# google-deepmind/mujoco_warp

Measured on NVIDIA H100. Metric: env-steps/sec (whole box) on humanoid.xml at nworld=8192 per GPU, higher is better.
Workload: dtype f32

## Files before the change

### mujoco_warp_b200/csrc/k_velocity.cu

```cuda

#include "mjb_fluid.cuh"
#include "mjb_math.cuh"
#include "mjb_muscle.cuh"
#include "mjb_team.cuh"
#include "mjb_types.cuh"

namespace {

struct VelLayout { int qvel, cdof, cinert, cvel, cdofdot, cacc, cfrc, qpas, qbias, qact, qsm, qld, x, af, total; };
__host__ __device__ inline VelLayout vel_layout(const ModelDev& m) {
  VelLayout L;
  int o = 0;
  auto pad = [](int n) { return (n + 3) & ~3; };
  auto take = [&](int n) { int r = o; o += pad(n); return r; };
  L.qpas = take(m.nv); L.qbias = take(m.nv);
  L.qsm = L.qpas; L.x = L.qbias;
  const int a0 = o;
  L.cdof = take(6 * m.nv); L.cinert = take(10 * m.nbody); L.qvel = take(m.nv);
  L.cvel = take(6 * m.nbody); L.cdofdot = take(6 * (m.nv > m.nbody ? m.nv : m.nbody)); L.cacc = take(6 * m.nbody);
  L.cfrc = L.cdofdot;
  if (pad(m.nv) + pad(m.nu) <= L.cvel - L.cinert) { L.qact = L.cinert; L.af = L.cinert + pad(m.nv); }
  else { L.qact = take(m.nv); L.af = take(m.nu); }
  L.qld = a0;
  if (o - a0 < pad(m.qld_total)) o = a0 + pad(m.qld_total);
  L.total = o;
  return L;
}

template <int LPW>
__device__ __forceinline__ void team_chol_upper(float* U, int n, float* x, bool solve, int sub) {
#pragma unroll 1
  for (int j = 0; j < n; j++) {
    const int iend = solve ? n + 1 : n;
#pragma unroll 1
    for (int i = j + sub; i < iend; i += LPW) {
      const bool rhs = i == n;
      const float* col = rhs ? x : U + i;
      const int cs = rhs ? 1 : n;
      float s0 = rhs ? x[j] : U[j * n + i], s1 = 0.f;
      int k = 0;
#pragma unroll 4
      for (; k + 1 < j; k += 2) {
        s0 -= U[k * n + j] * col[k * cs];
        s1 -= U[(k + 1) * n + j] * col[(k + 1) * cs];
      }
      if (k < j) s0 -= U[k * n + j] * col[k * cs];
      if (rhs) x[j] = s0 + s1; else U[j * n + i] = s0 + s1;
    }
    __syncwarp();
    const float piv = sqrtf(fmaxf(U[j * n + j], MJ_MINVAL)), inv = 1.0f / piv;
    __syncwarp();
#pragma unroll 1
    for (int i = j + sub; i < iend; i += LPW) {
      if (i == n) x[j] *= inv;
      else U[j * n + i] = i == j ? piv : U[j * n + i] * inv;
    }
    __syncwarp();
  }
  if (!solve) return;
#pragma unroll 1
  for (int j = n - 1; j >= 0; j--) {
    const float xj = x[j] / U[j * n + j];
    __syncwarp();
#pragma unroll 1
    for (int k = sub; k < j; k += LPW) x[k] -= U[k * n + j] * xj;
    if (sub == 0) x[j] = xj;
    __syncwarp();
  }
}

template <bool PEXT, int LPW, bool BAT>
__global__ void __launch_bounds__(256)
k_velocity(const __grid_constant__ ModelDev mp, const __grid_constant__ DataDev d, int mask) {
  constexpr bool FLUID = false;
  [[maybe_unused]] constexpr FluidDev f{};
#include "k_velocity_body.cuh"
}

template <int LPW, bool BAT>
__global__ void __launch_bounds__(256)
k_velocity_fluid(const __grid_constant__ ModelDev mp, const __grid_constant__ DataDev d, int mask, const __grid_constant__ FluidDev f) {
  constexpr bool PEXT = true, FLUID = true;
#include "k_velocity_body.cuh"
}

}

template <bool PEXT>
static TeamKernel vel_instance(int lpw, bool bat) {
  if (bat) return k_velocity<PEXT, 32, true>;
  return lpw == 8 ? k_velocity<PEXT, 8, false> : lpw == 16 ? k_velocity<PEXT, 16, false> : k_velocity<PEXT, 32, false>;
}
static bool vel_pext(const ModelDev& m) { return m.has_gravcomp || m.ntendon > 0; }
static TeamKernel vel_kernel(const ModelDev& m, int lpw) { return vel_pext(m) ? vel_instance<true>(lpw, m.batched) : vel_instance<false>(lpw, m.batched); }
using FluidKernel = void (*)(ModelDev, DataDev, int, FluidDev);
static FluidKernel vel_kernel_fluid(const ModelDev& m, int lpw) {
  if (m.batched) return k_velocity_fluid<32, true>;
  return lpw == 8 ? k_velocity_fluid<8, false> : lpw == 16 ? k_velocity_fluid<16, false> : k_velocity_fluid<32, false>;
}

size_t smem_velocity(const ModelDev& m, const DataDev& d, const FluidDev& f) {
  const int words = vel_layout(m).total;
  return f.has_fluid ? team_shape(m, d.wn, words, vel_kernel_fluid).block_bytes : team_shape(m, d.wn, words, vel_kernel).block_bytes;
}
cudaError_t launch_velocity(const ModelDev& m, const DataDev& d, int mask, cudaStream_t s, const FluidDev& f) {
  const int words = vel_layout(m).total;
  return f.has_fluid ? team_launch(m, d, words, vel_kernel_fluid, mask, s, f) : team_launch(m, d, words, vel_kernel, mask, s);
}
cudaError_t resident_worlds_velocity(const ModelDev& m, const DataDev& d, int* worlds, int* shape, const FluidDev& f) {
  const int words = vel_layout(m).total;
  shape[3] = f.has_fluid ? 2 : vel_pext(m) ? 1 : 0;
  return f.has_fluid ? team_resident_worlds(m, d, words, vel_kernel_fluid, worlds, shape) : team_resident_worlds(m, d, words, vel_kernel, worlds, shape);
}
```

### mujoco_warp_b200/csrc/k_velocity_body.cuh

```cuda
  extern __shared__ __align__(16) float smem[];
  constexpr int G = 32 / LPW;
  Team<LPW> T;
  T.init(d.w0, d.wn, d.nworld);
  if (T.nvalid <= 0) return;
  MJB_WORLD_MODEL(T.w)
  const int lane = T.lane, sub = T.sub, g = T.g, nval = T.nvalid;
  const bool valid = T.valid;
  const VelLayout L = vel_layout(mp);
  float* S = smem + (size_t)(threadIdx.x >> 5) * ((size_t)L.total * G + 4);
  Stager st;
  st.init(reinterpret_cast<uint64_t*>(S + (size_t)L.total * G), lane);
  const int nv = m.nv, nb = m.nbody, nu = m.nu;
#define FLD(f, n) (S + (size_t)L.f * G + (size_t)g * (n))
  float *qvel = FLD(qvel, nv), *cdof = FLD(cdof, 6 * nv), *cinert = FLD(cinert, 10 * nb), *cvel = FLD(cvel, 6 * nb), *cdofdot = FLD(cdofdot, 6 * nv),
        *cacc = FLD(cacc, 6 * nb), *cfrc = FLD(cfrc, 6 * nb), *q_passive = FLD(qpas, nv), *q_bias = FLD(qbias, nv), *q_act = FLD(qact, nv),
        *q_smooth = FLD(qsm, nv), *qld = FLD(qld, m.qld_total), *x = FLD(x, nv), *aforce = FLD(af, nu);
  const float* Mw = d.M + (size_t)T.w * m.nC;
#undef FLD
  const size_t wg = (size_t)T.wg0;
#define GLOAD(f, field, n) st.load(S + (size_t)L.f * G, d.field + wg * (size_t)(n), nval * (n))
#define GSTORE(field, f, n) st.store(d.field + wg * (size_t)(n), S + (size_t)L.f * G, nval * (n))
  const size_t wb = (size_t)T.w;
  const bool v_all = mask & STG_VELOCITY;

  GLOAD(qvel, qvel, nv); GLOAD(cdof, cdof, 6 * nv);
  if (v_all || (mask & STG_RNE)) GLOAD(cinert, cinert, 10 * nb);
  constexpr int MREG = 32;
  float mreg[MREG];
  const bool fac = mask & (STG_ACCELERATION | STG_FACTOR_ONLY);
#pragma unroll
  for (int k = 0; k < MREG; k++) { const int e = sub + k * LPW; mreg[k] = (fac && e < m.nC) ? Mw[e] : 0.f; }
  bool any_xfrc = false;
  if (mask & STG_ACCELERATION) {
#pragma unroll 4
    for (int i = sub; i < 6 * nb; i += LPW) any_xfrc |= d.xfrc_applied[wb * 6 * nb + i] != 0.f;
  }
  st.load_wait();

  if (mask & (STG_VELOCITY | STG_COMVEL | STG_PASSIVE | STG_RNE)) {
    if (v_all)
#pragma unroll 1
    for (int a = valid ? sub : nu; a < nu; a += LPW) {
      const int nnz = d.moment_rownnz[wb * nu + a], adr = d.moment_rowadr[wb * nu + a];
      float vel = 0.f;
      for (int k = 0; k < nnz; k++) vel += d.actuator_moment[wb * m.nJmom + adr + k] * qvel[d.moment_colind[wb * m.nJmom + adr + k]];
      d.actuator_velocity[wb * nu + a] = vel;
    }
    if (PEXT && v_all && m.ntendon > 0) {
#pragma unroll 1
      for (int t = valid ? sub : m.ntendon; t < m.ntendon; t += LPW) {
        float vel = 0.f;
        for (int k = m.ten_J_rowadr[t]; k < m.ten_J_rowadr[t] + m.ten_J_rownnz[t]; k++) vel += m.ten_J0[k] * qvel[m.ten_J_colind[k]];
        d.ten_velocity[wb * m.ntendon + t] = vel;
      }
    }
    if (v_all || (mask & STG_COMVEL)) {
    if (sub < 6) cvel[sub] = 0.f;
    __syncwarp();
#pragma unroll 1
    for (int l = 1; l < m.nlevel; l++) {
#pragma unroll 1
      for (int i = m.level_adr[l] + sub; i < m.level_adr[l + 1]; i += LPW) {
        const int b = m.level_body[i], pid = m.body_parentid[b], jntadr = m.body_jntadr[b], jntnum = m.body_jntnum[b];
        int dof = m.body_dofadr[b];
        float cv[6];
#pragma unroll
        for (int k = 0; k < 6; k++) cv[k] = cvel[6 * pid + k];
#pragma unroll 1
        for (int j = jntadr; j < jntadr + jntnum; j++) {
          const int t = m.jnt_type[j];
          if (t == JNT_FREE) {
            for (int q = 0; q < 3; q++) { const float v = qvel[dof + q]; for (int k = 0; k < 6; k++) { cv[k] += cdof[6 * (dof + q) + k] * v; cdofdot[6 * (dof + q) + k] = 0.f; } }
            for (int q = 3; q < 6; q++) motion_cross(cv, cdof + 6 * (dof + q), cdofdot + 6 * (dof + q));
            for (int q = 3; q < 6; q++) { const float v = qvel[dof + q]; for (int k = 0; k < 6; k++) cv[k] += cdof[6 * (dof + q) + k] * v; }
            dof += 6;
          } else if (t == JNT_BALL) {
            for (int q = 0; q < 3; q++) motion_cross(cv, cdof + 6 * (dof + q), cdofdot + 6 * (dof + q));
            for (int q = 0; q < 3; q++) { const float v = qvel[dof + q]; for (int k = 0; k < 6; k++) cv[k] += cdof[6 * (dof + q) + k] * v; }
            dof += 3;
          } else {
            motion_cross(cv, cdof + 6 * dof, cdofdot + 6 * dof);
            const float v = qvel[dof];
            for (int k = 0; k < 6; k++) cv[k] += cdof[6 * dof + k] * v;
            dof += 1;
          }
        }
#pragma unroll
        for (int k = 0; k < 6; k++) cvel[6 * b + k] = cv[k];
      }
      __syncwarp();
    }
    st.store_fence();
    GSTORE(cvel, cvel, 6 * nb); GSTORE(cdof_dot, cdofdot, 6 * nv);
    st.store_commit();
    } else if (mask & STG_RNE) {
      GLOAD(cvel, cvel, 6 * nb); GLOAD(cdofdot, cdof_dot, 6 * nv);
      st.load_wait();
    }

    if (v_all || (mask & STG_PASSIVE)) {
      const bool dsbl_spring = m.disableflags & DSBL_SPRING, dsbl_damper = m.disableflags & DSBL_DAMPER;
      const bool gravcomp = PEXT && m.has_gravcomp && !(m.disableflags & DSBL_GRAVITY) && !(dsbl_spring && dsbl_damper);
      [[maybe_unused]] const bool fluid = FLUID && !(dsbl_spring && dsbl_damper);
      if constexpr (FLUID) if (fluid) {
        const float* cv = (v_all || (mask & STG_COMVEL)) ? cvel : d.cvel + wb * 6 * nb;
        const float *xip = d.xipos + wb * nb * 3, *stc = d.subtree_com + wb * nb * 3;
#pragma unroll 1
        for (int b = sub; b < nb; b += LPW)
          fluid_body_wrench(m, f, b, cv + 6 * b, ld3(xip + 3 * b), d.ximat + (wb * nb + b) * 9, ld3(stc + 3 * m.body_rootid[b]), d.geom_xpos + wb * m.ngeom * 3,
                            d.geom_xmat + wb * m.ngeom * 9, cacc + 6 * b);
        __syncwarp();
      }
#pragma unroll 1
      for (int dd = sub; dd < nv; dd += LPW) {
        const int j = m.dof_jntid[dd], t = m.jnt_type[j];
        float spring = 0.f, damper = 0.f, gc = 0.f;
        if (!(dsbl_spring && dsbl_damper)) {
          const float stiffness = m.jnt_stiffness[j];
          if (stiffness != 0.f && !dsbl_spring) {
            const int qa = m.jnt_qposadr[j], k = dd - m.jnt_dofadr[j];
            if (t == JNT_SLIDE || t == JNT_HINGE) spring = -(d.qpos[wb * m.nq + qa] - m.qpos_spring[qa]) * stiffness;
            else if (!PEXT) {}
            else if (t == JNT_FREE && k < 3) spring = -stiffness * (d.qpos[wb * m.nq + qa + k] - m.qpos_spring[qa + k]);
            else {
              const int ra = t == JNT_FREE ? qa + 3 : qa, kk = t == JNT_FREE ? k - 3 : k;
              const q4 rot = qnormalize(ldq(d.qpos + wb * m.nq + ra)), ref = ldq(m.qpos_spring + ra);
              const q4 qd = qmul(mkq(ref.w, -ref.x, -ref.y, -ref.z), rot);
              const float s2 = sqrtf(qd.x * qd.x + qd.y * qd.y + qd.z * qd.z);
              if (s2 != 0.f) {
                float speed = 2.0f * atan2f(s2, qd.w);
                if (speed > 3.14159265358979f) speed -= 2.0f * 3.14159265358979f;
                spring = -stiffness * (kk == 0 ? qd.x : kk == 1 ? qd.y : qd.z) * (speed / s2);
              }
            }
          }
          const float damping = m.dof_damping[dd];
          if (damping != 0.f && !dsbl_damper) damper = -qvel[dd] * damping;
          if (PEXT && m.ntendon > 0) {
#pragma unroll 1
            for (int tn = 0; tn < m.ntendon; tn++) {
              const float ks = m.tendon_stiffness[tn], kd = m.tendon_damping[tn];
              if ((ks == 0.f || dsbl_spring) && (kd == 0.f || dsbl_damper)) continue;
              const float J = tendon_J_at(m, tn, dd);
              if (J == 0.f) continue;
              if (ks != 0.f && !dsbl_spring) {
                const float len = d.ten_length[wb * m.ntendon + tn], lo = m.tendon_lengthspring[2 * tn], hi = m.tendon_lengthspring[2 * tn + 1];
                const float x = len > hi ? len - hi : (len < lo ? len - lo : 0.f);
                spring += J * (-x * ks);
              }
              if (kd != 0.f && !dsbl_damper) {
                float vel = 0.f;
                for (int k = m.ten_J_rowadr[tn]; k < m.ten_J_rowadr[tn] + m.ten_J_rownnz[tn]; k++) vel += m.ten_J0[k] * qvel[m.ten_J_colind[k]];
                damper += J * (-vel * kd);
              }
            }
          }
        }
        if (gravcomp) {
#pragma unroll 1
          for (int b = 1; b < nb; b++) {
            const float g = m.body_gravcomp[b];
            if (g == 0.f || !m.body_isdofancestor[b * nv + dd]) continue;
            const float sc = -m.body_mass[b] * g;
            const v3 off = ld3(d.xipos + (wb * nb + b) * 3) - ld3(d.subtree_com + (wb * nb + m.body_rootid[b]) * 3);
            const v3 jp = ld3(cdof + 6 * dd + 3) + cross(ld3(cdof + 6 * dd), off);
            gc += sc * (jp.x * m.gravity_x + jp.y * m.gravity_y + jp.z * m.gravity_z);
          }
        }
        float passive = spring + damper + (m.jnt_actgravcomp[j] ? 0.f : gc);
        if constexpr (FLUID) {
          const float fl = fluid ? fluid_project(m, dd, cdof + 6 * dd, cacc, d.xipos + wb * nb * 3, d.subtree_com + wb * nb * 3) : 0.f;
          passive += fl;
          if (valid) f.qfrc_fluid[wb * nv + dd] = fl;
        }
        q_passive[dd] = passive;
        if (valid) {
          d.qfrc_spring[wb * nv + dd] = spring;
          d.qfrc_damper[wb * nv + dd] = damper;
          d.qfrc_gravcomp[wb * nv + dd] = gc;
          d.qfrc_passive[wb * nv + dd] = passive;
        }
      }
    }
    if (v_all || (mask & STG_RNE)) {
    for (int k = sub; k < 6; k += LPW) cacc[k] = k < 3 ? 0.f : ((m.disableflags & DSBL_GRAVITY) ? 0.f : -(k == 3 ? m.gravity_x : k == 4 ? m.gravity_y : m.gravity_z));
    __syncwarp();
#pragma unroll 1
    for (int l = 1; l < m.nlevel; l++) {
#pragma unroll 1
      for (int i = m.level_adr[l] + sub; i < m.level_adr[l + 1]; i += LPW) {
        const int b = m.level_body[i], pid = m.body_parentid[b];
        float a[6];
#pragma unroll
        for (int k = 0; k < 6; k++) a[k] = cacc[6 * pid + k];
#pragma unroll 1
        for (int q = 0; q < m.body_dofnum[b]; q++) {
          const int dof = m.body_dofadr[b] + q;
          const float v = qvel[dof];
#pragma unroll
          for (int k = 0; k < 6; k++) a[k] += cdofdot[6 * dof + k] * v;
        }
#pragma unroll
        for (int k = 0; k < 6; k++) cacc[6 * b + k] = a[k];
      }
      __syncwarp();
    }
    st.store_wait_read();
#pragma unroll 2
    for (int b = sub; b < nb; b += LPW) {
      float f[6] = {0.f, 0.f, 0.f, 0.f, 0.f, 0.f};
      if (b > 0) {
        float iv[6], g[6];
        inert_vec(cinert + 10 * b, cacc + 6 * b, f);
        inert_vec(cinert + 10 * b, cvel + 6 * b, iv);
        motion_cross_force(cvel + 6 * b, iv, g);
#pragma unroll
        for (int k = 0; k < 6; k++) f[k] += g[k];
      }
#pragma unroll
      for (int k = 0; k < 6; k++) cfrc[6 * b + k] = f[k];
    }
    __syncwarp();
#pragma unroll 1
    for (int l = m.nlevel - 2; l >= 0; l--) {
#pragma unroll 1
      for (int i = m.level_adr[l] + sub; i < m.level_adr[l + 1]; i += LPW) {
        const int b = m.level_body[i];
        float acc[6];
#pragma unroll
        for (int k = 0; k < 6; k++) acc[k] = cfrc[6 * b + k];
#pragma unroll 1
        for (int c = m.body_childadr[b]; c < m.body_childadr[b + 1]; c++) {
          const float* cc = cfrc + 6 * m.body_childid[c];
#pragma unroll
          for (int k = 0; k < 6; k++) acc[k] += cc[k];
        }
#pragma unroll
        for (int k = 0; k < 6; k++) cfrc[6 * b + k] = acc[k];
      }
      __syncwarp();
    }
#pragma unroll 1
    for (int dd = sub; dd < nv; dd += LPW) {
      const float v = dot6(cdof + 6 * dd, cfrc + 6 * m.dof_bodyid[dd]);
      q_bias[dd] = v;
    }
    st.store_fence();
    GSTORE(cacc, cacc, 6 * nb); GSTORE(cfrc_int, cfrc, 6 * nb); GSTORE(qfrc_bias, qbias, nv);
    st.store_commit();
    }
  } else if (mask & STG_ACCELERATION) {
    GLOAD(qpas, qfrc_passive, nv); GLOAD(qbias, qfrc_bias, nv);
    st.load_wait();
  }
  __syncwarp();

  if (mask & STG_ACTUATION) {
#pragma unroll 1
    for (int dd = sub; dd < nv; dd += LPW) q_act[dd] = 0.f;
    __syncwarp();
    const bool enabled = nu > 0 && !(m.disableflags & DSBL_ACTUATION);
#pragma unroll 1
    for (int a = sub; a < nu; a += LPW) {
      float force = 0.f;
      if (enabled) {
        float ctrl = d.ctrl[wb * nu + a];
        if (m.actuator_ctrllimited[a] && !(m.disableflags & DSBL_CLAMPCTRL)) ctrl = clampf(ctrl, m.actuator_ctrlrange[2 * a], m.actuator_ctrlrange[2 * a + 1]);
        const float length = d.actuator_length[wb * nu + a], velocity = d.actuator_velocity[wb * nu + a];
        const float *gp = m.actuator_gainprm + 10 * a, *bp = m.actuator_biasprm + 10 * a;
        float gain = 0.f, bias = 0.f;
        if (m.actuator_gaintype[a] == GAIN_FIXED) gain = gp[0];
        else if (m.actuator_gaintype[a] == GAIN_AFFINE) gain = gp[0] + gp[1] * length + gp[2] * velocity;
        else if (m.actuator_gaintype[a] == GAIN_MUSCLE)
          gain = muscle_gain(length, velocity, m.actuator_lengthrange[2 * a], m.actuator_lengthrange[2 * a + 1], m.actuator_acc0[a], gp);
        if (m.actuator_biastype[a] == BIAS_AFFINE) bias = bp[0] + bp[1] * length + bp[2] * velocity;
        else if (m.actuator_biastype[a] == BIAS_MUSCLE)
          bias = muscle_bias(length, m.actuator_lengthrange[2 * a], m.actuator_lengthrange[2 * a + 1], m.actuator_acc0[a], bp);
        float ctrl_act = ctrl;
        if (m.na > 0 && m.actuator_actadr[a] >= 0) {
          const int last = m.actuator_actadr[a] + m.actuator_actnum[a] - 1, dyn = m.actuator_dyntype[a];
          const float act = d.act[wb * m.na + last];
          float act_dot = 0.f;
          if (dyn == DYN_INTEGRATOR) act_dot = ctrl;
          else if (dyn == DYN_FILTER || dyn == DYN_FILTEREXACT) act_dot = (ctrl - act) / fmaxf(m.actuator_dynprm[10 * a], MJ_MINVAL);
          else if (dyn == DYN_MUSCLE) act_dot = muscle_dynamics(ctrl, act, m.actuator_dynprm + 10 * a);
          if (valid) d.act_dot[wb * m.na + last] = act_dot;
          ctrl_act = m.actuator_actearly[a] ? next_act(m, a, act, act_dot, 1.0f, m.actuator_actlimited[a] != 0) : act;
        }
        force = gain * ctrl_act + bias;
        if (m.actuator_forcelimited[a]) force = clampf(force, m.actuator_forcerange[2 * a], m.actuator_forcerange[2 * a + 1]);
      } else if (m.na > 0 && m.actuator_actadr[a] >= 0 && valid) {
        d.act_dot[wb * m.na + m.actuator_actadr[a] + m.actuator_actnum[a] - 1] = 0.f;
      }
      if (valid) d.actuator_force[wb * nu + a] = force;
      aforce[a] = force;
    }
    __syncwarp();
    if (PEXT && enabled && m.ntendon > 0) {
#pragma unroll 1
      for (int t = sub; t < m.ntendon; t += LPW) {
        if (!m.tendon_actfrclimited[t]) continue;
        float total = 0.f;
        for (int b = 0; b < nu; b++) if (m.actuator_trntype[b] == TRN_TENDON && m.actuator_trnid[2 * b] == t) total += aforce[b];
        const float lo = m.tendon_actfrcrange[2 * t], hi = m.tendon_actfrcrange[2 * t + 1];
        const float sc = total < lo ? lo / total : (total > hi ? hi / total : 1.0f);
        if (sc == 1.0f) continue;
        for (int b = 0; b < nu; b++)
          if (m.actuator_trntype[b] == TRN_TENDON && m.actuator_trnid[2 * b] == t) { aforce[b] *= sc; if (valid) d.actuator_force[wb * nu + b] = aforce[b]; }
      }
      __syncwarp();
    }
    if (enabled) {
#pragma unroll 1
      for (int dd = sub; dd < nv; dd += LPW) {
        float q = 0.f;
        for (int k = m.dofact_adr[dd]; k < m.dofact_adr[dd + 1]; k++) q += d.actuator_moment[wb * m.nJmom + m.dofact_mom[k]] * aforce[m.dofact_act[k]];
        const int j = m.dof_jntid[dd];
        if (!(m.disableflags & DSBL_GRAVITY) && m.jnt_actgravcomp[j]) q += d.qfrc_gravcomp[wb * nv + dd];
        if (m.jnt_actfrclimited[j]) q = clampf(q, m.jnt_actfrcrange[2 * j], m.jnt_actfrcrange[2 * j + 1]);
        q_act[dd] = q;
      }
    }
    st.store_fence();
    GSTORE(qfrc_actuator, qact, nv);
    st.store_commit();
  } else if (mask & STG_ACCELERATION) {
    GLOAD(qact, qfrc_actuator, nv);
    st.load_wait();
  }
  __syncwarp();

  if (mask & (STG_ACCELERATION | STG_FACTOR_ONLY)) {
    if (mask & STG_ACCELERATION) {
#pragma unroll 1
      for (int dd = sub; dd < nv; dd += LPW) q_smooth[dd] = q_passive[dd] - q_bias[dd] + q_act[dd] + d.qfrc_applied[wb * nv + dd];
      if (team_any<LPW>(any_xfrc, g)) {
#pragma unroll 1
        for (int dd = sub; dd < nv; dd += LPW) {
#include "k_body_xfrc.cuh"
          q_smooth[dd] += acc;
        }
      }
      __syncwarp();
    }
    const bool acc = mask & STG_ACCELERATION;
    st.store_wait_read();
#pragma unroll 1
    for (int i = sub; i < m.qld_total; i += LPW) qld[i] = 0.f;
    if (acc)
#pragma unroll 1
      for (int i = sub; i < nv; i += LPW) x[i] = q_smooth[i];
    __syncwarp();
#pragma unroll 1
    for (int t = 0; t < m.ntree; t++) {
      const int start = m.tree_dofadr[t], n = m.tree_dofnum[t];
      float* U = qld + m.tree_qLDadr[t];
      const int e0 = m.M_rowadr[start], e1 = m.M_rowadr[start + n - 1] + m.M_rownnz[start + n - 1];
#pragma unroll
      for (int k = 0; k < MREG; k++) {
        const int e = sub + k * LPW;
        if (e >= e0 && e < e1) U[(m.M_colind[e] - start) * n + (m.M_entry_row[e] - start)] = mreg[k];
      }
#pragma unroll 1
      for (int e = max(e0, MREG * LPW) + ((sub - max(e0, MREG * LPW)) % LPW + LPW) % LPW; e < e1; e += LPW)
        U[(m.M_colind[e] - start) * n + (m.M_entry_row[e] - start)] = Mw[e];
      __syncwarp();
      team_chol_upper<LPW>(U, n, x + start, acc, sub);
    }
    st.store_fence();
    if (acc) { GSTORE(qfrc_smooth, qsm, nv); GSTORE(qacc_smooth, x, nv); }
    GSTORE(qLD, qld, m.qld_total);
    st.store_commit();
  }
  st.store_wait_read();
#undef GLOAD
#undef GSTORE
```

Before: 20.63 million.

## Block the team Cholesky factorization and solve four columns at a time

```diff
diff --git a/mujoco_warp_b200/csrc/k_velocity.cu b/mujoco_warp_b200/csrc/k_velocity.cu
--- a/mujoco_warp_b200/csrc/k_velocity.cu
+++ b/mujoco_warp_b200/csrc/k_velocity.cu
@@ -27,44 +27,121 @@
   return L;
 }
 
+template <int LPW, int TT>
+__device__ __forceinline__ void chol_rows4(float* U, int n, float* x, int iend, int j0, int nb, int c0, int sub, bool first, float (&inv)[4],
+                                           float (&mul)[4][4]) {
+  const int base = (threadIdx.x & 31) - sub, xo = (int)(x - U);
+  int o[TT], s[TT], col[TT];
+  float acc[4][TT];
+#pragma unroll
+  for (int t = 0; t < TT; t++) {
+    const int i = c0 + sub + LPW * t;
+    col[t] = i;
+    o[t] = i < n ? i : i == n ? xo : 0;
+    s[t] = i < n ? n : i == n ? 1 : 0;
+#pragma unroll
+    for (int r = 0; r < 4; r++) acc[r][t] = r < nb ? U[o[t] + (j0 + r) * s[t]] : 0.f;
+  }
+  const float* uk = U + j0;
+#pragma unroll 2
+  for (int k = 0; k < j0; k++, uk += n) {
+    float a[4];
+#pragma unroll
+    for (int r = 0; r < 4; r++) a[r] = uk[r];
+#pragma unroll
+    for (int t = 0; t < TT; t++) {
+      const float b = U[o[t]];
+      o[t] += s[t];
+#pragma unroll
+      for (int r = 0; r < 4; r++) acc[r][t] -= a[r] * b;
+    }
+  }
+#pragma unroll
+  for (int r = 0; r < 4; r++) {
+    if (r < nb) {
+#pragma unroll
+      for (int q = 0; q < r; q++)
+#pragma unroll
+        for (int t = 0; t < TT; t++) acc[r][t] -= mul[q][r] * acc[q][t];
+      float piv = 0.f;
+      if (first) {
+        const float d = fmaxf(__shfl_sync(FULL_MASK, acc[r][0], base + r), MJ_MINVAL);
+        inv[r] = rsqrtf(d);
+        piv = d * inv[r];
+      }
+#pragma unroll
+      for (int t = 0; t < TT; t++) acc[r][t] = col[t] == j0 + r ? piv : acc[r][t] * inv[r];
+      if (first)
+#pragma unroll
+        for (int q = r + 1; q < 4; q++) mul[r][q] = __shfl_sync(FULL_MASK, acc[r][0], base + q);
+    }
+  }
+#pragma unroll
+  for (int r = 0; r < 4; r++) {
+#pragma unroll
+    for (int t = 0; t < TT; t++) {
+      const int i = col[t];
+      if (r < nb && i >= j0 + r && i < iend) {
+        if (i < n) U[(j0 + r) * n + i] = acc[r][t];
+        else x[j0 + r] = acc[r][t];
+      }
+    }
+  }
+}
+
 template <int LPW>
 __device__ __forceinline__ void team_chol_upper(float* U, int n, float* x, bool solve, int sub) {
+  constexpr int T = 32 / LPW;
+  const int iend = solve ? n + 1 : n;
+  float inv[4] = {0.f, 0.f, 0.f, 0.f}, mul[4][4] = {};
 #pragma unroll 1
-  for (int j = 0; j < n; j++) {
-    const int iend = solve ? n + 1 : n;
+  for (int j0 = 0; j0 < n; j0 += 4) {
+    const int nb = min(4, n - j0);
 #pragma unroll 1
-    for (int i = j + sub; i < iend; i += LPW) {
-      const bool rhs = i == n;
-      const float* col = rhs ? x : U + i;
-      const int cs = rhs ? 1 : n;
-      float s0 = rhs ? x[j] : U[j * n + i], s1 = 0.f;
-      int k = 0;
-#pragma unroll 4
-      for (; k + 1 < j; k += 2) {
-        s0 -= U[k * n + j] * col[k * cs];
-        s1 -= U[(k + 1) * n + j] * col[(k + 1) * cs];
+    for (int c0 = j0; c0 < iend; c0 += 32) {
+      const int tt = (min(32, iend - c0) + LPW - 1) / LPW;
+      const bool first = c0 == j0;
+      if constexpr (T == 4) {
+        if (tt == 4) chol_rows4<LPW, 4>(U, n, x, iend, j0, nb, c0, sub, first, inv, mul);
+        else if (tt == 3) chol_rows4<LPW, 3>(U, n, x, iend, j0, nb, c0, sub, first, inv, mul);
+        else if (tt == 2) chol_rows4<LPW, 2>(U, n, x, iend, j0, nb, c0, sub, first, inv, mul);
+        else chol_rows4<LPW, 1>(U, n, x, iend, j0, nb, c0, sub, first, inv, mul);
+      } else if constexpr (T == 2) {
+        if (tt == 2) chol_rows4<LPW, 2>(U, n, x, iend, j0, nb, c0, sub, first, inv, mul);
+        else chol_rows4<LPW, 1>(U, n, x, iend, j0, nb, c0, sub, first, inv, mul);
+      } else {
+        chol_rows4<LPW, 1>(U, n, x, iend, j0, nb, c0, sub, first, inv, mul);
       }
-      if (k < j) s0 -= U[k * n + j] * col[k * cs];
-      if (rhs) x[j] = s0 + s1; else U[j * n + i] = s0 + s1;
-    }
-    __syncwarp();
-    const float piv = sqrtf(fmaxf(U[j * n + j], MJ_MINVAL)), inv = 1.0f / piv;
-    __syncwarp();
-#pragma unroll 1
-    for (int i = j + sub; i < iend; i += LPW) {
-      if (i == n) x[j] *= inv;
-      else U[j * n + i] = i == j ? piv : U[j * n + i] * inv;
     }
     __syncwarp();
   }
   if (!solve) return;
 #pragma unroll 1
-  for (int j = n - 1; j >= 0; j--) {
-    const float xj = x[j] / U[j * n + j];
+  for (int j0 = (n - 1) & ~3; j0 >= 0; j0 -= 4) {
+    const int nb = min(4, n - j0);
+    float xb[4];
+#pragma unroll
+    for (int r = 3; r >= 0; r--) {
+      if (r < nb) {
+        float v = x[j0 + r];
+#pragma unroll
+        for (int q = 3; q > r; q--)
+          if (q < nb) v -= U[(j0 + r) * n + j0 + q] * xb[q];
+        xb[r] = v / U[(j0 + r) * n + j0 + r];
+      } else {
+        xb[r] = 0.f;
+      }
+    }
     __syncwarp();
 #pragma unroll 1
-    for (int k = sub; k < j; k += LPW) x[k] -= U[k * n + j] * xj;
-    if (sub == 0) x[j] = xj;
+    for (int k = sub; k < j0; k += LPW) {
+      float v = x[k];
+#pragma unroll
+      for (int q = 3; q >= 0; q--)
+        if (q < nb) v -= U[k * n + j0 + q] * xb[q];
+      x[k] = v;
+    }
+    if (sub < nb) x[j0 + sub] = xb[sub];
     __syncwarp();
   }
 }
diff --git a/mujoco_warp_b200/csrc/k_velocity_body.cuh b/mujoco_warp_b200/csrc/k_velocity_body.cuh
--- a/mujoco_warp_b200/csrc/k_velocity_body.cuh
+++ b/mujoco_warp_b200/csrc/k_velocity_body.cuh
@@ -364,9 +364,10 @@
 #pragma unroll 1
       for (int e = max(e0, MREG * LPW) + ((sub - max(e0, MREG * LPW)) % LPW + LPW) % LPW; e < e1; e += LPW)
         U[(m.M_colind[e] - start) * n + (m.M_entry_row[e] - start)] = Mw[e];
-      __syncwarp();
-      team_chol_upper<LPW>(U, n, x + start, acc, sub);
-    }
+    }
+    __syncwarp();
+#pragma unroll 1
+    for (int t = 0; t < m.ntree; t++) team_chol_upper<LPW>(qld + m.tree_qLDadr[t], m.tree_dofnum[t], x + m.tree_dofadr[t], acc, sub);
     st.store_fence();
     if (acc) { GSTORE(qfrc_smooth, qsm, nv); GSTORE(qacc_smooth, x, nv); }
     GSTORE(qLD, qld, m.qld_total);
```

Result: faster. 21.18 million (median of 6 runs) (+2.7%).
